# MegviiRobot/CamLaserCalibraTool

Hardware: NVIDIA H100
Metric: residual+Jacobian evals/sec (full LM solves) (higher is better)
Workload: dtype f64

## Files before the change

camlasercalibratool_b200/csrc/clc_api.cu:

```cuda
#include <cuda_runtime.h>
#include <dlfcn.h>
#include <nccl.h>

#include <algorithm>
#include <atomic>
#include <chrono>
#include <cmath>
#include <cstddef>
#include <cstdio>
#include <cstdlib>
#include <cstring>
#include <functional>
#include <mutex>
#include <string>
#include <vector>

#include "../../include/clc_b200.h"
#include "clc_kernels.cuh"
#include "clc_l2_plan.h"
#include "clc_linefit.cuh"
#include "clc_small.cuh"
#include "clc_subset.cuh"
#include "clc_subset_plan.h"
#include "clc_trim.cuh"
// ... 128 lines not shown
    if (piv != k) {
      for (int j = 0; j < n; ++j) std::swap(A[k * n + j], A[piv * n + j]);
      for (int j = 0; j < n; ++j) std::swap(A[j * n + k], A[j * n + piv]);
      std::swap(b[k], b[piv]);
      std::swap(perm[k], perm[piv]);
    }
    const double d = A[k * n + k];
    if (d == 0.0) continue;
    for (int i = k + 1; i < n; ++i) {
      const double l = A[i * n + k] / d;
      for (int j = k + 1; j < n; ++j) A[i * n + j] -= l * A[k * n + j];
      A[i * n + k] = l;
    }
  }
  double z[9], y[9];
  for (int i = 0; i < n; ++i) {
    double s = b[i];
    for (int k = 0; k < i; ++k) s -= A[i * n + k] * z[k];
    z[i] = s;
  }
  for (int i = 0; i < n; ++i) z[i] = (A[i * n + i] != 0.0) ? z[i] / A[i * n + i] : 0.0;
  for (int i = n - 1; i >= 0; --i) {
    double s = z[i];
    for (int k = i + 1; k < n; ++k) s -= A[k * n + i] * y[k];
    y[i] = s;
  }
  for (int i = 0; i < n; ++i) x[perm[i]] = y[i];
}

int64_t round_up(int64_t v, int64_t m) { return (v + m - 1) / m * m; }

}

struct PinnedBlock {
  clc::LmState lm;
  double sums[clc::kMaxOut];
  double pose[8];
  int done;
  int nonplanar;
};
namespace {
std::mutex g_pinned_mutex;
std::vector<PinnedBlock*> g_pinned_free;
PinnedBlock* pinned_acquire() {
  {
    std::lock_guard<std::mutex> lock(g_pinned_mutex);
    if (!g_pinned_free.empty()) {
      PinnedBlock* b = g_pinned_free.back();
      g_pinned_free.pop_back();
      return b;
    }
  }
  PinnedBlock* b = nullptr;
  if (cudaMallocHost(&b, sizeof(PinnedBlock)) != cudaSuccess) return nullptr;
  return b;
}
void pinned_release(PinnedBlock* b) {
  if (!b) return;
  std::lock_guard<std::mutex> lock(g_pinned_mutex);
  g_pinned_free.push_back(b);
}
}

struct clc_comm {
  ncclComm_t comm = nullptr;
  int nranks = 1, rank = 0, device = 0;
  void* p2p_block = nullptr;
  void* peer_block[clc::kMaxRanks] = {};
  bool p2p_ready = false;
  bool local = false;
  size_t mailbox_bytes() const { return sizeof(unsigned long long) * 2 * 2 * (size_t)nranks * clc::kMailboxSlot; }
  size_t block_bytes() const { return mailbox_bytes() + sizeof(unsigned long long); }
};

struct clc_problem {
  int device = 0;
  cudaStream_t stream = nullptr;
  int num_sms = 0;
  int64_t l2_bytes = 0;
  int grid = 0;
  int64_t n_frames = 0, n_points = 0, n_points_padded = 0, n_edges = 0;
  int use_loss = 1;
  double cauchy_a = 0.05;
  double *x = nullptr, *y = nullptr, *z = nullptr;
  void *xy_block = nullptr, *z_block = nullptr;
  double* frame_pose = nullptr;
  double* frame_pose_true = nullptr;
  double* plane = nullptr;
  int64_t* offsets = nullptr;
  int* warp_first_frame = nullptr;
  double* edge_plane = nullptr;
  double* edge_pt = nullptr;
  unsigned long long* partials_ll = nullptr;
  unsigned int* launch_seq = nullptr;
  unsigned long long* pose_ll = nullptr;
  double* sums = nullptr;
  double* pose = nullptr;
  clc::LmState* lm = nullptr;
  double* flush_buf = nullptr;
  int64_t flush_n = 0;
  unsigned long long* timing = nullptr;
  bool use_pdl = true;
  int64_t l2_persist_bytes = 0;
  bool l2_window_set = false;
  int64_t l2_resident_bytes = -1;
  int resident_chunks = 0;
  bool small_kernel = true;
  int loop_in_kernel = 1;
  PinnedBlock* pinned = nullptr;
  double* h_sums = nullptr;
  int* h_done = nullptr;
  clc::LmState* h_lm = nullptr;
  clc_comm* comm_obj = nullptr;
  ncclComm_t comm = nullptr;
  int nranks = 1, rank = 0;
  int* p2p_error = nullptr;
  int allreduce_mode = 0;
  int64_t per_warp = 0;
  int grid_full = 0;
  cudaEvent_t ev0 = nullptr, ev1 = nullptr;
  int* d_nonplanar = nullptr;
  bool z_all_zero = false;
  bool host_planarity_known = false;
  bool planar = false;
  int planar_mode = 1;
  int64_t planar_min_points = 0;
};

namespace {

clc::ProblemView make_view(const clc_problem* p) {
  clc::ProblemView v;
  v.x = p->x; v.y = p->y; v.z = p->z;
  v.plane = p->plane;
  v.offsets = p->offsets;
  v.warp_first_frame = p->warp_first_frame;
  v.edge_plane = p->edge_plane;
  v.edge_pt = p->edge_pt;
  v.n_frames = p->n_frames;
  v.n_points = p->n_points;
  v.n_edges = p->n_edges;
  v.per_warp = p->per_warp;
  v.resident_chunks = p->resident_chunks;
  v.a2 = p->cauchy_a * p->cauchy_a;
  v.inv_a2 = 1.0 / v.a2;
  return v;
}

int set_device(const clc_problem* p) {
  CLC_CUDA(cudaSetDevice(p->device));
  return CLC_OK;
}

int launch_sweep(clc_problem* p, int mode, bool loss, bool edges, const double* d_pose, const int* d_done,
                 clc::LmState* d_lm, bool collective = true, bool pdl = false, int loop_sweeps = 1, bool l2_hints = false,
                 double* frame_rows = nullptr, double* frame_slots = nullptr) {
  clc::SweepArgs a;
  a.pose7 = d_pose;
  a.done = d_done;
  a.partials_ll = p->partials_ll;
  a.sums = p->sums;
  a.launch_seq = p->launch_seq;
  a.pose_ll = p->pose_ll;
  a.lm = d_lm;
  a.use_loss = loss ? 1 : 0;
  a.use_edges = edges ? 1 : 0;
  a.l2_hints = l2_hints ? 1 : 0;
  a.loop_sweeps = loop_sweeps;
  a.timing = p->timing;
  a.nranks = 1;
  a.rank = 0;
  a.seq_counter = nullptr;
  a.error = p->p2p_error;
  a.frame_rows = frame_rows;
  a.frame_slots = frame_slots;
  if (p->nranks > 1 && p->allreduce_mode == 1 && collective) {
    clc_comm* c = p->comm_obj;
    a.nranks = c->nranks;
    a.rank = c->rank;
    a.seq_counter = reinterpret_cast<unsigned long long*>(static_cast<char*>(c->p2p_block) + c->mailbox_bytes());
    for (int r = 0; r < c->nranks; ++r) a.peer_mailbox[r] = static_cast<unsigned long long*>(c->peer_block[r]);
  }
  const clc::ProblemView v = make_view(p);
  cudaLaunchConfig_t cfg = {};
  cfg.gridDim = dim3((unsigned)p->grid);
  cfg.blockDim = dim3(clc::kThreads);
  cfg.dynamicSmemBytes = mode == clc::kModeFrames ? clc::frames_smem_bytes(p->planar) : clc::dyn_smem_bytes(p->planar);
  cfg.stream = p->stream;
  cudaLaunchAttribute attr[1];
  attr[0].id = cudaLaunchAttributeProgrammaticStreamSerialization;
  attr[0].val.programmaticStreamSerializationAllowed = pdl ? 1 : 0;
  cfg.attrs = attr;
  cfg.numAttrs = 1;
  cudaError_t le;
  if (!p->planar && p->z == nullptr) return fail(CLC_ERR_INVALID, "internal: general sweep without a z stream");
  if (mode == clc::kModeFrames) {
    if (frame_rows == nullptr || frame_slots == nullptr || d_lm != nullptr || loop_sweeps > 1 || a.nranks > 1)
      return fail(CLC_ERR_INVALID, "internal: bad per-frame sweep");
    void (*fn)(clc::ProblemView, clc::SweepArgs) =
        loss ? (p->planar ? clc::clc_sweep_kernel<true, clc::kModeFrames, true> : clc::clc_sweep_kernel<true, clc::kModeFrames, false>)
             : (p->planar ? clc::clc_sweep_kernel<false, clc::kModeFrames, true> : clc::clc_sweep_kernel<false, clc::kModeFrames, false>);
    CLC_CUDA(cudaFuncSetAttribute(fn, cudaFuncAttributeMaxDynamicSharedMemorySize, (int)cfg.dynamicSmemBytes));
    le = cudaLaunchKernelEx(&cfg, fn, v, a);
  } else if (mode == clc::kModeClosedForm) {
    le = p->planar ? cudaLaunchKernelEx(&cfg, clc::clc_sweep_kernel<false, clc::kModeClosedForm, true>, v, a)
                   : cudaLaunchKernelEx(&cfg, clc::clc_sweep_kernel<false, clc::kModeClosedForm, false>, v, a);
  } else if (loop_sweeps > 1) {
    if (d_lm == nullptr) return fail(CLC_ERR_INVALID, "internal: looping sweep without an LM state");
    if (loss)
      le = p->planar ? cudaLaunchKernelEx(&cfg, clc::clc_sweep_kernel<true, clc::kModeLM, true, true>, v, a)
                     : cudaLaunchKernelEx(&cfg, clc::clc_sweep_kernel<true, clc::kModeLM, false, true>, v, a);
    else
      le = p->planar ? cudaLaunchKernelEx(&cfg, clc::clc_sweep_kernel<false, clc::kModeLM, true, true>, v, a)
                     : cudaLaunchKernelEx(&cfg, clc::clc_sweep_kernel<false, clc::kModeLM, false, true>, v, a);
  } else if (loss) {
    le = p->planar ? cudaLaunchKernelEx(&cfg, clc::clc_sweep_kernel<true, clc::kModeLM, true>, v, a)
                   : cudaLaunchKernelEx(&cfg, clc::clc_sweep_kernel<true, clc::kModeLM, false>, v, a);
  } else {
    le = p->planar ? cudaLaunchKernelEx(&cfg, clc::clc_sweep_kernel<false, clc::kModeLM, true>, v, a)
                   : cudaLaunchKernelEx(&cfg, clc::clc_sweep_kernel<false, clc::kModeLM, false>, v, a);
  }
  if (le != cudaSuccess) return fail(CLC_ERR_CUDA, std::string("sweep launch: ") + cudaGetErrorString(le));
  CLC_LAUNCH_CHECK();
  return CLC_OK;
}

int allreduce_sums(clc_problem* p, int count) {
  if (p->nranks <= 1 || p->allreduce_mode == 1) return CLC_OK;
  CLC_NCCL(nccl_api()->AllReduce(p->sums, p->sums, (size_t)count, ncclDouble, ncclSum, p->comm, p->stream));
  return CLC_OK;
}

cudaError_t sync_stream_low_latency(cudaStream_t st) {
  const auto t0 = std::chrono::steady_clock::now();
  for (;;) {
    const cudaError_t e = cudaStreamQuery(st);
    if (e != cudaErrorNotReady) return e;
    if (std::chrono::steady_clock::now() - t0 > std::chrono::microseconds(400)) return cudaStreamSynchronize(st);
#if defined(__x86_64__) || defined(__i386__)
    __builtin_ia32_pause();
#endif
  }
}

int check_p2p_error(clc_problem* p) {
  if (p->grid <= 1 && p->nranks <= 1) return CLC_OK;
  int err = 0;
  CLC_CUDA(cudaMemcpyAsync(&err, p->p2p_error, sizeof(int), cudaMemcpyDeviceToHost, p->stream));
  CLC_CUDA(sync_stream_low_latency(p->stream));
  if (err == 2) return fail(CLC_ERR_CUDA, "sweep kernel: the persistent grid was not co-resident (ticket wait timed out)");
  if (err) return fail(CLC_ERR_NCCL, "peer exchange timed out: a rank did not reach the collective");
  return CLC_OK;
}

int materialise_z(clc_problem* p);

int partition(clc_problem* p) {
  const int chunk = p->planar ? clc::kPlanarChunk : clc::kChunk;
  p->grid = p->grid_full;
  {
    const int64_t stages = (p->n_points + chunk - 1) / chunk;
    const int64_t blocks_needed = std::max<int64_t>(1, (stages + clc::kWarps - 1) / clc::kWarps);
    if (blocks_needed < p->grid) p->grid = (int)blocks_needed;
    int64_t single_block_max = (int64_t)clc::kWarps * 8 * clc::kChunk;
    if (const char* env = std::getenv("CLC_SINGLE_BLOCK_MAX_POINTS")) single_block_max = std::atoll(env);
    if (p->n_points <= single_block_max) p->grid = 1;
  }
  const int64_t n_warps = (int64_t)p->grid * clc::kWarps;
  p->per_warp = std::max<int64_t>(chunk, round_up((p->n_points + n_warps - 1) / n_warps, chunk));
  if (p->warp_first_frame) CLC_CUDA(cudaFreeAsync(p->warp_first_frame, p->stream));
  if (p->partials_ll) CLC_CUDA(cudaFreeAsync(p->partials_ll, p->stream));
  p->warp_first_frame = nullptr;
  p->partials_ll = nullptr;
  CLC_CUDA(cudaMallocAsync(&p->warp_first_frame, sizeof(int) * n_warps, p->stream));
  const size_t ll_bytes = sizeof(unsigned long long) * 2 * (size_t)p->grid * clc::kMaxOut;
  CLC_CUDA(cudaMallocAsync(&p->partials_ll, ll_bytes, p->stream));
  {
    const int64_t stage_bytes = (int64_t)(p->planar ? 2 : 3) * chunk * 8;
    const bool latency_bound = p->n_points <= clc::kSmallMaxResiduals;
    const int64_t budget = p->l2_persist_bytes > 0 ? 0 : clc::l2_resident_budget(p->l2_bytes, p->l2_resident_bytes);
    p->resident_chunks = clc::l2_resident_chunks(budget, p->grid, clc::kWarps, p->per_warp / chunk, stage_bytes, latency_bound);
  }
  CLC_CUDA(cudaMemsetAsync(p->partials_ll, 0, ll_bytes, p->stream));
  const int threads = 256;
  const int blocks = (int)((n_warps + threads - 1) / threads);
  clc::clc_warp_table_kernel<<<blocks, threads, 0, p->stream>>>(p->offsets, p->n_frames, p->n_points, p->per_warp, n_warps,
                                                                p->warp_first_frame);
  CLC_LAUNCH_CHECK();
  return CLC_OK;
}

int finish_create(clc_problem* p) {
  const int threads = 256;
  if (p->n_frames > 0) {
    const int blocks = (int)((p->n_frames + threads - 1) / threads);
    clc::clc_planes_kernel<<<blocks, threads, 0, p->stream>>>(p->frame_pose, p->n_frames, p->plane, p->edge_plane);
    CLC_LAUNCH_CHECK();
  }
  static std::mutex cfg_mutex;
  static int cached_blocks_per_sm[64] = {};
  int blocks_per_sm = 0;
  {
    std::lock_guard<std::mutex> lock(cfg_mutex);
    if (p->device < 64) blocks_per_sm = cached_blocks_per_sm[p->device];
  }
  if (blocks_per_sm == 0) {
    int occ = 0, occ_min = 1 << 30;
    const void* variants[] = {
        (const void*)clc::clc_sweep_kernel<true, clc::kModeLM, false>,         (const void*)clc::clc_sweep_kernel<true, clc::kModeLM, true>,
        (const void*)clc::clc_sweep_kernel<false, clc::kModeLM, false>,        (const void*)clc::clc_sweep_kernel<false, clc::kModeLM, true>,
        (const void*)clc::clc_sweep_kernel<false, clc::kModeClosedForm, false>, (const void*)clc::clc_sweep_kernel<false, clc::kModeClosedForm, true>,
        (const void*)clc::clc_sweep_kernel<true, clc::kModeLM, false, true>,   (const void*)clc::clc_sweep_kernel<true, clc::kModeLM, true, true>,
        (const void*)clc::clc_sweep_kernel<false, clc::kModeLM, false, true>,  (const void*)clc::clc_sweep_kernel<false, clc::kModeLM, true, true>};
    for (int v = 0; v < 10; ++v) {
      const void* fn = variants[v];
      const int smem = clc::dyn_smem_bytes((v & 1) != 0);
      CLC_CUDA(cudaFuncSetAttribute(fn, cudaFuncAttributeMaxDynamicSharedMemorySize, smem));
      CLC_CUDA(cudaOccupancyMaxActiveBlocksPerMultiprocessor(&occ, fn, clc::kThreads, smem));
      occ_min = std::min(occ_min, occ);
    }
    if (occ_min < 1) return fail(CLC_ERR_CUDA, "the sweep kernel does not fit on this device");
// ... 2345 lines not shown
```

camlasercalibratool_b200/csrc/clc_kernels.cuh:

```cuda
#pragma once

#include <cuda_runtime.h>

#include "clc_camera.cuh"
#include "clc_expand.cuh"
#include "clc_frames.cuh"
#include "clc_lm.cuh"

namespace clc {

#ifndef CLC_THREADS
#define CLC_THREADS 384
#endif
#ifndef CLC_BLOCKS_PER_SM
#define CLC_BLOCKS_PER_SM 1
#endif
#ifndef CLC_STAGES
#define CLC_STAGES 2
#endif
constexpr int kThreads = CLC_THREADS;
constexpr int kBlocksPerSM = CLC_BLOCKS_PER_SM;
constexpr int kWarps = kThreads / 32;
constexpr int kTileStride = 13;
#ifndef CLC_CHUNK
#define CLC_CHUNK 128
#endif
constexpr int kChunk = CLC_CHUNK;
constexpr int kGroups = kChunk / 64;
constexpr int kStages = CLC_STAGES;
constexpr int kMaxOut = 54;
constexpr int kMaxRanks = 16;
constexpr int kMailboxSlot = 64;
#ifndef CLC_PLANAR_STAGES
#define CLC_PLANAR_STAGES CLC_STAGES
#endif
#ifndef CLC_PLANAR_CHUNK
#define CLC_PLANAR_CHUNK (CLC_CHUNK * 2)
#endif
constexpr int kPlanarStages = CLC_PLANAR_STAGES;
constexpr int kPlanarChunk = CLC_PLANAR_CHUNK;
static_assert(kChunk % 64 == 0 && kPlanarChunk % 64 == 0, "stages are made of 64-point groups");
constexpr int kMaxChunk = kChunk > kPlanarChunk ? kChunk : kPlanarChunk;
#ifndef CLC_LOCKSTEP_SLACK
#define CLC_LOCKSTEP_SLACK 0
#endif
constexpr int kLockstepSlack = CLC_LOCKSTEP_SLACK;
constexpr int kBarsPerWarp = kStages > kPlanarStages ? kStages : kPlanarStages;
constexpr int kTileDoublesPerWarp = 32 * kTileStride;
__host__ __device__ constexpr int ring_doubles_per_warp(bool planar) { return planar ? kPlanarStages * 2 * kPlanarChunk : kStages * 3 * kChunk; }
__host__ __device__ constexpr int dyn_smem_bytes(bool planar) {
  return kWarps * ring_doubles_per_warp(planar) * 8 + kWarps * kTileDoublesPerWarp * 8 + kWarps * kBarsPerWarp * 8;
}

constexpr int kFrameTileDoublesPerWarp = 32 * 3;
__host__ __device__ constexpr int frames_smem_bytes(bool planar) {
  return dyn_smem_bytes(planar) + kWarps * kFrameTileDoublesPerWarp * 8;
}

enum SweepMode { kModeLM = 0, kModeClosedForm = 1, kModeFrames = 2 };

struct ProblemView {
  const double* x;
  const double* y;
  const double* z;
  const double* plane;
  const int64_t* offsets;
  const int* warp_first_frame;
  const double* edge_plane;
  const double* edge_pt;
  int64_t n_frames;
  int64_t n_points;
  int64_t n_edges;
  int64_t per_warp;
  int resident_chunks;
  double inv_a2;
  double a2;
};

struct SweepArgs {
  const double* pose7;
  const int* done;
  unsigned long long* partials_ll;
  double* sums;
  unsigned int* launch_seq;
  LmState* lm;
  int use_loss;
  int use_edges;
  int l2_hints;
  int loop_sweeps;
  unsigned long long* pose_ll;
  unsigned long long* timing;
  int nranks;
  int rank;
  unsigned long long* seq_counter;
  unsigned long long* peer_mailbox[kMaxRanks];
  int* error;
  double* frame_rows;
  double* frame_slots;
};


__device__ __forceinline__ unsigned long long globaltimer_ns() {
  unsigned long long t;
  asm volatile("mov.u64 %0, %globaltimer;" : "=l"(t));
  return t;
}
#define CLC_STAMP(slot)                                                                       \
  do {                                                                                        \
    if (args.timing != nullptr && threadIdx.x == 0) args.timing[(int64_t)blockIdx.x * 8 + (slot)] = globaltimer_ns(); \
  } while (0)

__device__ __forceinline__ uint32_t smem_u32(const void* p) { return (uint32_t)__cvta_generic_to_shared(p); }

__device__ __forceinline__ void mbar_init(uint64_t* bar, uint32_t count) {
  asm volatile("mbarrier.init.shared::cta.b64 [%0], %1;" ::"r"(smem_u32(bar)), "r"(count) : "memory");
}
__device__ __forceinline__ void mbar_expect_tx(uint64_t* bar, uint32_t bytes) {
  asm volatile("mbarrier.arrive.expect_tx.shared::cta.b64 _, [%0], %1;" ::"r"(smem_u32(bar)), "r"(bytes) : "memory");
}
__device__ __forceinline__ void mbar_wait(uint64_t* bar, uint32_t parity) {
  uint32_t done;
  do {
    asm volatile(
        "{\n\t.reg .pred p;\n\t"
        "mbarrier.try_wait.parity.shared::cta.b64 p, [%1], %2;\n\t"
        "selp.u32 %0, 1, 0, p;\n\t}"
        : "=r"(done)
        : "r"(smem_u32(bar)), "r"(parity)
        : "memory");
  } while (!done);
}
__device__ __forceinline__ void bulk_g2s(void* dst, const void* src, uint32_t bytes, uint64_t* bar) {
  asm volatile("cp.async.bulk.shared::cluster.global.mbarrier::complete_tx::bytes [%0], [%1], %2, [%3];" ::"r"(
                   smem_u32(dst)),
               "l"(src), "r"(bytes), "r"(smem_u32(bar))
               : "memory");
}
__device__ __forceinline__ void bulk_g2s_hint(void* dst, const void* src, uint32_t bytes, uint64_t* bar, uint64_t policy) {
  asm volatile("cp.async.bulk.shared::cluster.global.mbarrier::complete_tx::bytes.L2::cache_hint [%0], [%1], %2, [%3], %4;" ::"r"(
                   smem_u32(dst)),
               "l"(src), "r"(bytes), "r"(smem_u32(bar)), "l"(policy)
               : "memory");
}
__device__ __forceinline__ uint64_t policy_evict_last() {
  uint64_t pol;
  asm("createpolicy.fractional.L2::evict_last.b64 %0, 1.0;" : "=l"(pol));
  return pol;
}
__device__ __forceinline__ uint64_t policy_evict_first() {
  uint64_t pol;
  asm("createpolicy.fractional.L2::evict_first.b64 %0, 1.0;" : "=l"(pol));
  return pol;
}

__device__ __forceinline__ void st_relaxed_sys(unsigned long long* p, unsigned long long v) {
  asm volatile("st.relaxed.sys.global.u64 [%0], %1;" ::"l"(p), "l"(v) : "memory");
}
__device__ __forceinline__ unsigned long long ld_relaxed_sys(const unsigned long long* p) {
  unsigned long long v;
  asm volatile("ld.relaxed.sys.global.u64 %0, [%1];" : "=l"(v) : "l"(p) : "memory");
  return v;
}

__device__ __forceinline__ void st_volatile_v2(unsigned long long* p, unsigned long long a, unsigned long long b) {
  asm volatile("st.volatile.global.v2.u64 [%0], {%1, %2};" ::"l"(p), "l"(a), "l"(b) : "memory");
}
__device__ __forceinline__ void ld_volatile_v2(const unsigned long long* p, unsigned long long& a, unsigned long long& b) {
  asm volatile("ld.volatile.global.v2.u64 {%0, %1}, [%2];" : "=l"(a), "=l"(b) : "l"(p) : "memory");
}

__device__ __forceinline__ unsigned int ld_acquire_gpu(const unsigned int* p) {
  unsigned int v;
  asm volatile("ld.acquire.gpu.global.u32 %0, [%1];" : "=r"(v) : "l"(p) : "memory");
  return v;
}
__device__ __forceinline__ unsigned int atom_add_acq_rel_gpu(unsigned int* p, unsigned int v) {
  unsigned int old;
  asm volatile("atom.acq_rel.gpu.global.add.u32 %0, [%1], %2;" : "=r"(old) : "l"(p), "r"(v) : "memory");
  return old;
}

__device__ __forceinline__ double rcp_pos(double a) {
  double r;
  asm("rcp.approx.ftz.f64 %0, %1;" : "=d"(r) : "d"(a));
  double e = fma(-a, r, 1.0);
  r = fma(r, e, r);
  e = fma(-a, r, 1.0);
  r = fma(r, e, r);
  return r;
}

__device__ __forceinline__ double warp_sum(double v) {
#pragma unroll
  for (int o = 16; o > 0; o >>= 1) v += __shfl_xor_sync(0xffffffffu, v, o);
  return v;
}

template <int N>
__device__ __forceinline__ void warp_transpose_sum(double* v, int lane) {
#pragma unroll
  for (int half = N / 2; half >= 1; half >>= 1) {
    const bool upper = (lane & half) != 0;
#pragma unroll
    for (int i = 0; i < half; ++i) {
      const double keep = upper ? v[i + half] : v[i];
      const double send = upper ? v[i] : v[i + half];
      v[i] = keep + __shfl_xor_sync(0xffffffffu, send, half);
    }
  }
#pragma unroll
  for (int o = N; o < 32; o <<= 1) v[0] += __shfl_xor_sync(0xffffffffu, v[0], o);
}

struct Moments {
  double S0, Sx, Sy, Sz, Sxx, Sxy, Sxz, Syy, Syz, Szz;
  double prod;
  int esum;
};

template <bool LOSS>
__device__ __forceinline__ void moments_clear(Moments& a) {
  a.S0 = a.Sx = a.Sy = a.Sz = a.Sxx = a.Sxy = a.Sxz = a.Syy = a.Syz = a.Szz = 0.0;
  a.prod = LOSS ? 1.0 : 0.0;
  a.esum = 0;
}

template <bool PLANAR>
__device__ __forceinline__ void accumulate(Moments& a, double w, double x, double y, double z) {
  const double wx = w * x, wy = w * y;
  a.S0 += w;
  a.Sx += wx; a.Sy += wy;
  a.Sxx = fma(wx, x, a.Sxx); a.Sxy = fma(wx, y, a.Sxy);
  a.Syy = fma(wy, y, a.Syy);
  if (!PLANAR) {
    const double wz = w * z;
    a.Sz += wz;
    a.Sxz = fma(wx, z, a.Sxz); a.Syz = fma(wy, z, a.Syz); a.Szz = fma(wz, z, a.Szz);
  }
}

template <bool LOSS, bool COST, bool PLANAR>
__device__ __forceinline__ void process2(Moments& a, const double2 X, const double2 Y, const double2 Z, bool v0,
                                         bool v1, double m0, double m1, double m2, double c, double inv_a2) {
  const double e0 = fma(m0, X.x, fma(m1, Y.x, PLANAR ? c : fma(m2, Z.x, c)));
  const double e1 = fma(m0, X.y, fma(m1, Y.y, PLANAR ? c : fma(m2, Z.y, c)));
  if (LOSS) {
    double u0 = fma(e0 * inv_a2, e0, 1.0);
    double u1 = fma(e1 * inv_a2, e1, 1.0);
    u0 = v0 ? u0 : 1.0;
    u1 = v1 ? u1 : 1.0;
    const double p = u0 * u1;
    const double r = rcp_pos(p);
    double w0 = r * u1, w1 = r * u0;
    w0 = v0 ? w0 : 0.0;
    w1 = v1 ? w1 : 0.0;
    a.prod *= p;
    accumulate<PLANAR>(a, w0, X.x, Y.x, Z.x);
    accumulate<PLANAR>(a, w1, X.y, Y.y, Z.y);
  } else {
    if (COST) {
      a.prod = fma(v0 ? e0 : 0.0, e0, a.prod);
      a.prod = fma(v1 ? e1 : 0.0, e1, a.prod);
    }
    accumulate<PLANAR>(a, v0 ? 1.0 : 0.0, X.x, Y.x, Z.x);
    accumulate<PLANAR>(a, v1 ? 1.0 : 0.0, X.y, Y.y, Z.y);
  }
}

__device__ __forceinline__ void renormalise(Moments& a) {
  const int hi = __double2hiint(a.prod);
  const int ex = (hi >> 20) - 1023;
  a.esum += ex;
  a.prod = __hiloint2double(hi - (ex << 20), __double2loint(a.prod));
}

struct FrameSums {
  double se, se2, emax;
};

__device__ __forceinline__ void frame_sums_clear(FrameSums& s) { s.se = s.se2 = s.emax = 0.0; }

template <bool PLANAR>
__device__ __forceinline__ void frame_sums2(FrameSums& s, const double2 X, const double2 Y, const double2 Z, bool v0, bool v1,
                                            double m0, double m1, double m2, double c) {
  const double e0 = fma(m0, X.x, fma(m1, Y.x, PLANAR ? c : fma(m2, Z.x, c)));
  const double e1 = fma(m0, X.y, fma(m1, Y.y, PLANAR ? c : fma(m2, Z.y, c)));
  const double d0 = v0 ? e0 : 0.0, d1 = v1 ? e1 : 0.0;
  s.se += d0;
  s.se += d1;
  s.se2 = fma(d0, d0, s.se2);
  s.se2 = fma(d1, d1, s.se2);
  s.emax = nan_max(s.emax, fabs(d0));
  s.emax = nan_max(s.emax, fabs(d1));
}

__device__ __forceinline__ void frame_row_write(const ProblemView& pv, const PoseConsts& pc, int64_t f, int64_t n, const double* S,
                                                double cost_term, double se, double se2, double emax, bool loss, bool edges,
                                                double* row) {
  double plane[4], m[3], c;
#pragma unroll
  for (int k = 0; k < 4; ++k) plane[k] = pv.plane[f * 4 + k];
  frame_consts(pc, plane, m, &c);
  const double s2 = 1.0 / (double)(pv.offsets[f + 1] - pv.offsets[f]);
  double out[kNumSums];
#pragma unroll
  for (int k = 0; k < kNumSums; ++k) out[k] = 0.0;
  expand_lm(plane, m, c, s2, S, loss, cost_term, pv.a2, out);
  double ee[2] = {0.0, 0.0};
  if (edges) {
#pragma unroll
    for (int k = 0; k < 2; ++k)
      ee[k] = edge_residual(pc, pv.edge_plane + (2 * f + k) * 4, pv.edge_pt + (2 * f + k) * 3, s2, loss, pv.a2, pv.inv_a2, out);
  }
  const double dn = (double)n;
  row[kRowN] = __longlong_as_double(n);
  row[kRowCost] = out[27];
  row[kRowChi] = s2 * se2;
  row[kRowMeanE] = se / dn;
  row[kRowRmsE] = sqrt(se2 / dn);
  row[kRowMaxE] = emax;
  row[kRowMeanW] = S[0] / dn;
  row[kRowEdgeE] = ee[0];
  row[kRowEdgeE + 1] = ee[1];
#pragma unroll
  for (int k = 0; k < 21; ++k) row[kRowH + k] = out[k];
#pragma unroll
  for (int k = 0; k < 6; ++k) row[kRowG + k] = out[21 + k];
}

template <bool LOSS, int MODE, bool PLANAR, bool LOOP = false>
__global__ void __launch_bounds__(kThreads, kBlocksPerSM)
clc_sweep_kernel(ProblemView pv, SweepArgs args) {
  constexpr int NOUT = (MODE == kModeClosedForm) ? kMaxOut : kNumSums;
  constexpr int NST = PLANAR ? kPlanarStages : kStages;
  constexpr int CH = PLANAR ? kPlanarChunk : kChunk;
  constexpr int G = CH / 64;
  constexpr int SST = (PLANAR ? 2 : 3) * CH;
  constexpr int RING = NST * SST;
  static_assert(RING == ring_doubles_per_warp(PLANAR), "ring size");
  extern __shared__ __align__(128) unsigned char s_dyn[];
  __shared__ double s_acc[kWarps][NOUT];
  __shared__ double s_red[kWarps][32];
  __shared__ unsigned long long s_core[kLmCoreWords];
  __shared__ double s_next[8];
  __shared__ int s_prog[32];

  CLC_STAMP(0);
  if (args.timing != nullptr && threadIdx.x == 0) {
    unsigned int smid;
    asm volatile("mov.u32 %0, %smid;" : "=r"(smid));
    args.timing[(int64_t)blockIdx.x * 8 + 7] = smid;
  }

  const int lane = threadIdx.x & 31;
  const int warp = threadIdx.x >> 5;
  const int64_t gwarp = (int64_t)blockIdx.x * kWarps + warp;

  const int64_t P = pv.n_points;
  int64_t p0 = gwarp * pv.per_warp;
  if (p0 > P) p0 = P;
  int64_t p1 = p0 + pv.per_warp;
  if (p1 > P) p1 = P;
  const int n_chunks = (int)((p1 - p0 + CH - 1) / CH);
  double* ring = reinterpret_cast<double*>(s_dyn) + warp * RING;
  double* tile = reinterpret_cast<double*>(s_dyn) + kWarps * RING + warp * kTileDoublesPerWarp;
  uint64_t* bars = reinterpret_cast<uint64_t*>(s_dyn + (size_t)kWarps * (RING + kTileDoublesPerWarp) * 8) + warp * kBarsPerWarp;
  double* ftile = reinterpret_cast<double*>(s_dyn + dyn_smem_bytes(PLANAR)) + warp * kFrameTileDoublesPerWarp;

  const int sweeps_max = (LOOP && args.loop_sweeps > 1 && MODE == kModeLM && args.lm != nullptr) ? args.loop_sweeps : 1;
  const int total_chunks = LOOP ? sweeps_max * n_chunks : n_chunks;
  int issued = 0, next_c = 0;
  const bool l2_hints = args.l2_hints != 0 && pv.resident_chunks > 0;
  auto issue_one = [&](bool slot_was_read) {
    if (lane == 0) {
      const int c = LOOP ? next_c : issued, st = issued % NST;
      double* dst = ring + st * SST;
      const int64_t src = p0 + (int64_t)c * CH;
      if (slot_was_read) asm volatile("fence.proxy.async.shared::cta;" ::: "memory");
      mbar_expect_tx(bars + st, (PLANAR ? 2 : 3) * CH * 8);
      if (l2_hints) {
        const uint64_t pol = c >= n_chunks - pv.resident_chunks ? policy_evict_last() : policy_evict_first();
        bulk_g2s_hint(dst, pv.x + src, CH * 8, bars + st, pol);
        bulk_g2s_hint(dst + CH, pv.y + src, CH * 8, bars + st, pol);
        if (!PLANAR) bulk_g2s_hint(dst + 2 * CH, pv.z + src, CH * 8, bars + st, pol);
      } else {
        bulk_g2s(dst, pv.x + src, CH * 8, bars + st);
        bulk_g2s(dst + CH, pv.y + src, CH * 8, bars + st);
        if (!PLANAR) bulk_g2s(dst + 2 * CH, pv.z + src, CH * 8, bars + st);
      }
    }
    ++issued;
    if (LOOP && ++next_c == n_chunks) next_c = 0;
  };
  auto drain = [&](int g) {
    for (; g < issued; ++g) mbar_wait(bars + g % NST, (uint32_t)(g / NST) & 1u);
  };
  if (lane == 0) {
#pragma unroll
    for (int st = 0; st < NST; ++st) mbar_init(bars + st, 1);
    asm volatile("fence.mbarrier_init.release.cluster;" ::: "memory");
    asm volatile("fence.proxy.async.shared::cta;" ::: "memory");
  }
  __syncwarp();
  for (int g = 0; g < NST && g < total_chunks; ++g) issue_one(false);
  __syncwarp();

  asm volatile("griddepcontrol.wait;" ::: "memory");
  if (args.done != nullptr && (*args.done != 0 || (args.error != nullptr && *args.error != 0))) {
    drain(0);
    return;
  }

  const unsigned int launch_tag0 = *args.launch_seq + 1u;
  if (MODE == kModeLM && args.lm != nullptr && blockIdx.x == 0) {
    const unsigned long long* g_core = reinterpret_cast<const unsigned long long*>(&args.lm->core);
    for (int k = threadIdx.x; k < kLmCoreWords; k += kThreads) s_core[k] = __ldcg(g_core + k);
  }

  PoseConsts pc;
  int n_tile = 0;

  auto flush_tile = [&]() {
    double out[NOUT];
#pragma unroll
    for (int k = 0; k < NOUT; ++k) out[k] = 0.0;
    __syncwarp();
    if (lane < n_tile) {
      const double* row = tile + lane * kTileStride;
      const int64_t f = __double_as_longlong(row[12]);
      double plane[4];
#pragma unroll
      for (int k = 0; k < 4; ++k) plane[k] = pv.plane[f * 4 + k];
      if (MODE == kModeLM) {
        double m[3], c;
        frame_consts(pc, plane, m, &c);
        const double cnt = (double)(pv.offsets[f + 1] - pv.offsets[f]);
        double cost_term = row[10];
        if (LOSS) cost_term = log(row[10]) + row[11] * 0.693147180559945309417232121458;
        expand_lm(plane, m, c, 1.0 / cnt, row, LOSS, cost_term, pv.a2, out);
      } else {
        expand_closed_form(plane, row, out);
      }
    }
    {
      double v[32];
#pragma unroll
      for (int k = 0; k < 32; ++k) v[k] = (k < NOUT) ? out[k] : 0.0;
      warp_transpose_sum<32>(v, lane);
      if (lane < NOUT) s_acc[warp][lane] += v[0];
      if (NOUT > 32) {
#pragma unroll
        for (int k = 0; k < 32; ++k) v[k] = (32 + k < NOUT) ? out[(32 + k < NOUT) ? 32 + k : 0] : 0.0;
        warp_transpose_sum<32>(v, lane);
        if (32 + lane < NOUT) s_acc[warp][32 + lane] += v[0];
      }
    }
    __syncwarp();
    n_tile = 0;
  };

  auto flush_frames = [&]() {
    __syncwarp();
    if (lane < n_tile) {
      const double* row = tile + lane * kTileStride;
      const double* rx = ftile + lane * 3;
      const int64_t f = __double_as_longlong(row[12]);
      const double cost_term = LOSS ? log(row[10]) + row[11] * 0.693147180559945309417232121458 : rx[1];
      frame_row_write(pv, pc, f, pv.offsets[f + 1] - pv.offsets[f], row, cost_term, rx[0], rx[1], rx[2], LOSS,
                      args.use_edges && pv.n_edges > 0, args.frame_rows + f * kRowDoubles);
    }
    __syncwarp();
    n_tile = 0;
  };

  int gc_base = 0;
  for (int sw = 0;; ++sw) {
  const unsigned int launch_tag = LOOP ? launch_tag0 + (unsigned int)sw : launch_tag0;
  for (int k = lane; k < NOUT; k += 32) s_acc[warp][k] = 0.0;
  {
    double pose[7];
#pragma unroll
    for (int i = 0; i < 7; ++i) pose[i] = (LOOP && sw > 0) ? s_next[i] : args.pose7[i];
    make_pose_consts(pose, &pc);
  }

  if (kLockstepSlack > 0) {
    if (lane == 0) s_prog[warp] = n_chunks > 0 ? 0 : 0x7fffffff;
    if (warp == 0 && lane >= kWarps) s_prog[lane] = 0x7fffffff;
    __syncthreads();
  }
  if (n_chunks > 0) {
    int64_t f = pv.warp_first_frame[gwarp];
    int64_t f_end = pv.offsets[f + 1];
    double m0 = 0.0, m1 = 0.0, m2 = 0.0, c = 0.0;
    double nx_plane[4] = {0.0, 0.0, 0.0, 0.0};
    int64_t nx_end = 0;
    auto prefetch_next = [&]() {
      if (f + 1 < pv.n_frames) {
#pragma unroll
        for (int k = 0; k < 4; ++k) nx_plane[k] = pv.plane[(f + 1) * 4 + k];
        nx_end = pv.offsets[f + 2];
      }
    };
    auto set_frame_consts = [&](const double* plane) {
      double m[3];
      frame_consts(pc, plane, m, &c);
      m0 = m[0]; m1 = m[1]; m2 = m[2];
    };
    {
      double plane[4];
#pragma unroll
      for (int k = 0; k < 4; ++k) plane[k] = pv.plane[f * 4 + k];
      set_frame_consts(plane);
      prefetch_next();
    }
    Moments a;
    moments_clear<LOSS>(a);
    bool open = false;
    FrameSums fx;
    frame_sums_clear(fx);
    int64_t piece_n = 0;

    auto park_piece = [&]() {
      double v[16] = {a.S0, a.Sx, a.Sy, a.Sz, a.Sxx, a.Sxy, a.Sxz, a.Syy, a.Syz, a.Szz, 0.0, 0.0, 0.0, 0.0, 0.0, 0.0};
      double pr = a.prod;
      int es = a.esum;
      double em = 0.0;
      if (MODE == kModeFrames) {
        v[12] = fx.se;
        v[13] = fx.se2;
        em = fx.emax;
#pragma unroll
        for (int o = 16; o > 0; o >>= 1) em = nan_max(em, __shfl_xor_sync(0xffffffffu, em, o));
      }
      if (LOSS) {
#pragma unroll
        for (int o = 16; o > 0; o >>= 1) {
          pr *= __shfl_xor_sync(0xffffffffu, pr, o);
          es += __shfl_xor_sync(0xffffffffu, es, o);
        }
      } else {
        v[10] = pr;
      }
      warp_transpose_sum<16>(v, lane);
      const int kind = MODE == kModeFrames ? frame_piece_kind(pv.offsets[f], f_end, p0, p1) : (int)kPieceWhole;
      if (kind != kPieceWhole) {
        double* slot = args.frame_slots + (gwarp * 2 + (kind == kPieceHead ? kSlotHead : kSlotTail)) * kSlotDoubles;
        if (lane < 10 || lane == 12 || lane == 13) slot[lane] = v[0];
        if (lane == 10) slot[10] = LOSS ? pr : 0.0;
        if (lane == 11) slot[11] = (double)es;
        if (lane == 14) slot[14] = em;
        if (lane == 15) slot[15] = (double)piece_n;
      } else {
        {
          double* row = tile + n_tile * kTileStride;
          if (lane < 10 || (!LOSS && lane == 10)) row[lane] = v[0];
          if (LOSS && lane == 10) row[10] = pr;
          if (lane == 11) row[11] = (double)es;
          if (lane == 12) row[12] = __longlong_as_double(f);
        }
        if (MODE == kModeFrames) {
          double* rx = ftile + n_tile * 3;
          if (lane == 12) rx[0] = v[0];
          if (lane == 13) rx[1] = v[0];
          if (lane == 14) rx[2] = em;
        }
        ++n_tile;
        if (n_tile == 32) {
          if (MODE == kModeFrames) flush_frames();
          else flush_tile();
        }
      }
      moments_clear<LOSS>(a);
      open = false;
      if (MODE == kModeFrames) {
        frame_sums_clear(fx);
        piece_n = 0;
      }
    };

    for (int ch = 0; ch < n_chunks; ++ch) {
      const int gc = LOOP ? gc_base + ch : ch;
      const int st = gc % NST;
      const int64_t cb = p0 + (int64_t)ch * CH;
      const int64_t ce = (cb + CH < p1) ? cb + CH : p1;
      if (kLockstepSlack > 0) {
        while (__reduce_min_sync(0xffffffffu, *(volatile int*)&s_prog[lane]) < ch - kLockstepSlack) __nanosleep(40);
      }
      mbar_wait(bars + st, (uint32_t)(gc / NST) & 1u);
      const double* sx = ring + st * SST;
      double2 X[G], Y[G], Z[G];
#pragma unroll
      for (int g = 0; g < G; ++g) {
        X[g] = *reinterpret_cast<const double2*>(sx + 64 * g + 2 * lane);
        Y[g] = *reinterpret_cast<const double2*>(sx + CH + 64 * g + 2 * lane);
        Z[g] = PLANAR ? make_double2(0.0, 0.0) : *reinterpret_cast<const double2*>(sx + 2 * CH + 64 * g + 2 * lane);
      }
      int64_t q = cb;
      while (q < ce) {
        while (f_end <= q) {
          ++f;
          if (nx_end > q) {
            f_end = nx_end;
            set_frame_consts(nx_plane);
          } else {
            f_end = pv.offsets[f + 1];
            if (f_end > q) {
              double plane[4];
#pragma unroll
              for (int k = 0; k < 4; ++k) plane[k] = pv.plane[f * 4 + k];
              set_frame_consts(plane);
            }
          }
          if (f_end > q) prefetch_next();
          else nx_end = 0;
        }
        const int64_t hi = f_end < ce ? f_end : ce;
        if (q == cb && hi == cb + CH) {
#pragma unroll
          for (int g = 0; g < G; ++g) {
            process2<LOSS, MODE == kModeLM, PLANAR>(a, X[g], Y[g], Z[g], true, true, m0, m1, m2, c, pv.inv_a2);
            if (MODE == kModeFrames) frame_sums2<PLANAR>(fx, X[g], Y[g], Z[g], true, true, m0, m1, m2, c);
          }
        } else {
#pragma unroll
          for (int g = 0; g < G; ++g) {
            const int64_t i0 = cb + 64 * g + 2 * lane;
            process2<LOSS, MODE == kModeLM, PLANAR>(a, X[g], Y[g], Z[g], i0 >= q && i0 < hi, i0 + 1 >= q && i0 + 1 < hi, m0, m1, m2,
                                            c, pv.inv_a2);
            if (MODE == kModeFrames)
              frame_sums2<PLANAR>(fx, X[g], Y[g], Z[g], i0 >= q && i0 < hi, i0 + 1 >= q && i0 + 1 < hi, m0, m1, m2, c);
          }
        }
        if (LOSS) renormalise(a);
        open = true;
        if (MODE == kModeFrames) piece_n += hi - q;
        q = hi;
        if (hi == f_end) park_piece();
      }
      __syncwarp();
      if (issued < total_chunks) issue_one(true);
      if (kLockstepSlack > 0 && lane == 0) *(volatile int*)&s_prog[warp] = (ch + 1 == n_chunks) ? 0x7fffffff : ch + 1;
    }
    if (open) park_piece();
  }
  if (MODE == kModeFrames) {
    flush_frames();
    return;
  }
  CLC_STAMP(1);
  if (args.timing != nullptr && lane == 0) args.timing[(int64_t)gridDim.x * 8 + gwarp] = globaltimer_ns();
  flush_tile();
  CLC_STAMP(2);

  if (MODE == kModeLM && args.use_edges && pv.n_edges > 0) {
    const int64_t total_lanes = (int64_t)gridDim.x * kThreads;
    double out[NOUT];
#pragma unroll
    for (int k = 0; k < NOUT; ++k) out[k] = 0.0;
    bool any = false;
    for (int64_t i = gwarp * 32 + lane; i < pv.n_edges; i += total_lanes) {
      const int64_t f = i >> 1;
      const int64_t cnt = pv.offsets[f + 1] - pv.offsets[f];
      if (cnt <= 0) continue;
      any = true;
      double plane[4], m[3], c;
#pragma unroll
      for (int k = 0; k < 4; ++k) plane[k] = pv.edge_plane[i * 4 + k];
      frame_consts(pc, plane, m, &c);
      const double x = pv.edge_pt[i * 3], y = pv.edge_pt[i * 3 + 1], z = pv.edge_pt[i * 3 + 2];
      const double e = fma(m[0], x, fma(m[1], y, fma(m[2], z, c)));
      double w = 1.0, cost_term = e * e;
      if (LOSS) {
        const double u = fma(e * pv.inv_a2, e, 1.0);
        w = 1.0 / u;
        cost_term = log(u);
      }
      const double S[10] = {w, w * x, w * y, w * z, w * x * x, w * x * y, w * x * z, w * y * y, w * y * z, w * z * z};
      expand_lm(plane, m, c, 1.0 / (double)cnt, S, LOSS, cost_term, pv.a2, out);
    }
    if (__any_sync(0xffffffffu, any)) {
      double v[32];
#pragma unroll
      for (int k = 0; k < 32; ++k) v[k] = (k < NOUT) ? out[k] : 0.0;
      warp_transpose_sum<32>(v, lane);
      if (lane < NOUT) s_acc[warp][lane] += v[0];
      __syncwarp();
    }
  }

  const unsigned long long ll_tag = (unsigned long long)launch_tag << 32;
  __syncthreads();
  double block_sum = 0.0;
  if (threadIdx.x < NOUT) {
#pragma unroll
    for (int wv = 0; wv < kWarps; ++wv) block_sum += s_acc[wv][threadIdx.x];
    if (gridDim.x > 1) {
      const unsigned long long bits = (unsigned long long)__double_as_longlong(block_sum);
      st_volatile_v2(args.partials_ll + ((int64_t)blockIdx.x * kMaxOut + threadIdx.x) * 2, ll_tag | (bits & 0xffffffffull),
                     ll_tag | (bits >> 32));
    }
  }
  CLC_STAMP(3);
  asm volatile("griddepcontrol.launch_dependents;" ::: "memory");
  if (blockIdx.x != 0 && (!LOOP || sweeps_max == 1)) return;

  if (blockIdx.x == 0) {
    constexpr int PARTS = kThreads / NOUT;
    constexpr int NB = 10;
    double* s_gather = &s_red[0][0];
    static_assert(kWarps * 32 >= PARTS * NOUT, "s_red holds one value per gathering thread");
    if (gridDim.x > 1 && threadIdx.x < PARTS * NOUT) {
      const int k = threadIdx.x % NOUT, part = threadIdx.x / NOUT;
      double acc = 0.0;
      for (int base = part; base < (int)gridDim.x; base += PARTS * NB) {
        unsigned long long w0[NB], w1[NB];
        unsigned int pending = 0u;
#pragma unroll
        for (int u = 0; u < NB; ++u)
          if (base + u * PARTS < (int)gridDim.x) pending |= 1u << u;
        unsigned int polls = 0;
        unsigned long long t0 = 0;
        while (pending != 0u) {
#pragma unroll
          for (int u = 0; u < NB; ++u)
            if ((pending >> u) & 1u)
              ld_volatile_v2(args.partials_ll + ((int64_t)(base + u * PARTS) * kMaxOut + k) * 2, w0[u], w1[u]);
#pragma unroll
          for (int u = 0; u < NB; ++u)
            if (((pending >> u) & 1u) && (w0[u] & 0xffffffff00000000ull) == ll_tag && (w1[u] & 0xffffffff00000000ull) == ll_tag)
              pending &= ~(1u << u);
          if (pending != 0u && (++polls & 0xffu) == 0u) {
            const unsigned long long now = globaltimer_ns();
            if (t0 == 0) t0 = now;
            else if (now - t0 > 2000000000ull) {
              if (args.error != nullptr) *args.error = 2;
              break;
            }
          }
        }
#pragma unroll
        for (int u = 0; u < NB; ++u)
          if (base + u * PARTS < (int)gridDim.x) acc += __longlong_as_double((long long)((w1[u] << 32) | (w0[u] & 0xffffffffull)));
      }
      s_gather[threadIdx.x] = acc;
    }
    double total = block_sum;
    if (gridDim.x > 1) {
      __syncthreads();
      total = 0.0;
      if (threadIdx.x < NOUT) {
#pragma unroll
        for (int part = 0; part < PARTS; ++part) total += s_gather[part * NOUT + threadIdx.x];
      }
    }
    if (args.nranks > 1) {
      double* s_tot = s_acc[0];
      double* s_x = reinterpret_cast<double*>(s_dyn) + kWarps * RING;
      static_assert(kWarps * kTileDoublesPerWarp >= kMaxRanks * kMaxOut, "the tiles hold one value per rank and output");
      __syncthreads();
      if (threadIdx.x < NOUT) s_tot[threadIdx.x] = total;
      __syncthreads();
      const unsigned long long seq = *args.seq_counter + 1ull;
      const unsigned long long tag = (seq & 0xffffffffull) << 32;
      const int par = (int)(seq & 1ull);
      const int n_words = args.nranks * NOUT;
      for (int idx = threadIdx.x; idx < n_words; idx += kThreads) {
        const int r = idx / NOUT, k = idx % NOUT;
        const unsigned long long bits = (unsigned long long)__double_as_longlong(s_tot[k]);
        const int64_t slot = (((int64_t)par * args.nranks + args.rank) * kMailboxSlot + k) * 2;
        st_relaxed_sys(args.peer_mailbox[r] + slot, tag | (bits & 0xffffffffull));
        st_relaxed_sys(args.peer_mailbox[r] + slot + 1, tag | (bits >> 32));
      }
      const unsigned long long t0 = globaltimer_ns();
      for (int idx = threadIdx.x; idx < n_words; idx += kThreads) {
        const int r = idx / NOUT, k = idx % NOUT;
        const unsigned long long* src = args.peer_mailbox[args.rank] + (((int64_t)par * args.nranks + r) * kMailboxSlot + k) * 2;
        unsigned long long a0, a1;
        unsigned int polls = 0;
        for (;;) {
          a0 = ld_relaxed_sys(src);
          a1 = ld_relaxed_sys(src + 1);
          if ((a0 & 0xffffffff00000000ull) == tag && (a1 & 0xffffffff00000000ull) == tag) break;
          if ((++polls & 0x3fu) == 0u && globaltimer_ns() - t0 > 5000000000ull) {
            if (args.error != nullptr) *args.error = 1;
            break;
          }
        }
        s_x[idx] = __longlong_as_double((long long)((a1 << 32) | (a0 & 0xffffffffull)));
      }
      __syncthreads();
      if (threadIdx.x < NOUT) {
        total = 0.0;
        for (int r = 0; r < args.nranks; ++r) total += s_x[r * NOUT + threadIdx.x];
      }
      if (threadIdx.x == 0) *args.seq_counter = seq;
    }
    __syncthreads();
    if (threadIdx.x < NOUT) {
      args.sums[threadIdx.x] = total;
      if (threadIdx.x < 32) s_red[0][threadIdx.x] = total;
    }
    __syncthreads();
    CLC_STAMP(4);
    if (threadIdx.x == 0) *args.launch_seq = launch_tag;
    if (MODE == kModeLM && args.lm != nullptr) {
      if (threadIdx.x == 0) {
        double sums[kNumSums];
        for (int k = 0; k < kNumSums; ++k) sums[k] = s_red[0][k];
        if (args.error != nullptr && *args.error != 0) {
          reinterpret_cast<LmCore*>(s_core)->done = CLC_TERM_FAILURE;
        } else {
          lm_update(reinterpret_cast<LmCore*>(s_core), args.lm->trace, sums);
        }
      }
      __syncthreads();
      if (LOOP && sweeps_max > 1 && threadIdx.x < 8) {
        const LmCore* core = reinterpret_cast<const LmCore*>(s_core);
        const double v = threadIdx.x < 7 ? core->cand[threadIdx.x] : (double)core->done;
        s_next[threadIdx.x] = v;
        if (gridDim.x > 1) {
          const unsigned long long bits = (unsigned long long)__double_as_longlong(v);
          st_volatile_v2(args.pose_ll + 2 * threadIdx.x, ll_tag | (bits & 0xffffffffull), ll_tag | (bits >> 32));
        }
      }
      unsigned long long* o_core = reinterpret_cast<unsigned long long*>(&args.lm->core);
      for (int k = threadIdx.x; k < kLmCoreWords; k += kThreads) o_core[k] = s_core[k];
    }
    CLC_STAMP(5);
  } else {
    if (threadIdx.x < 8 && sw + 1 < sweeps_max) {
      unsigned long long a0, a1, t0 = 0;
      unsigned int polls = 0;
      for (;;) {
        ld_volatile_v2(args.pose_ll + 2 * threadIdx.x, a0, a1);
        if ((a0 & 0xffffffff00000000ull) == ll_tag && (a1 & 0xffffffff00000000ull) == ll_tag) break;
        if ((++polls & 0xffu) == 0u) {
          const unsigned long long now = globaltimer_ns();
          if (t0 == 0) t0 = now;
          else if (now - t0 > 10000000000ull) {
            if (args.error != nullptr) *args.error = 2;
            a0 = a1 = 0;
            break;
          }
        }
      }
      const bool lost = (a0 | a1) == 0ull;
      s_next[threadIdx.x] = lost ? (double)CLC_TERM_FAILURE : __longlong_as_double((long long)((a1 << 32) | (a0 & 0xffffffffull)));
    }
  }
  if (!LOOP || sw + 1 >= sweeps_max) break;
  gc_base += n_chunks;
  __syncthreads();
  if (s_next[7] != 0.0) {
    drain(gc_base);
    break;
  }
  }
}

__global__ void clc_lm_kernel(LmState* lm, const double* sums) {
  if (threadIdx.x == 0 && blockIdx.x == 0) {
    double s[kNumSums];
    for (int k = 0; k < kNumSums; ++k) s[k] = sums[k];
    lm_update(&lm->core, lm->trace, s);
  }
}

template <bool LOSS>
__global__ void clc_frame_fixup_kernel(ProblemView pv, const double* pose7, int edges, const double* __restrict__ slots,
                                       double* __restrict__ rows) {
  const int64_t f = (int64_t)blockIdx.x * blockDim.x + threadIdx.x;
  if (f >= pv.n_frames) return;
  const int64_t fs = pv.offsets[f], fe = pv.offsets[f + 1];
  double* row = rows + f * kRowDoubles;
  if (fe <= fs) {
    for (int k = 0; k < kRowDoubles; ++k) row[k] = 0.0;
    return;
  }
  int64_t w0, w1;
  frame_warps(fs, fe, pv.per_warp, &w0, &w1);
  if (w0 == w1) return;
  double S[10] = {0.0, 0.0, 0.0, 0.0, 0.0, 0.0, 0.0, 0.0, 0.0, 0.0};
  double cost_term = 0.0, se = 0.0, se2 = 0.0, emax = 0.0;
  int64_t n = 0;
  for (int64_t w = w0; w <= w1; ++w) {
    const double* s = slots + frame_slot(w, w0);
#pragma unroll
    for (int k = 0; k < 10; ++k) S[k] += s[k];
    cost_term += LOSS ? log(s[10]) + s[11] * 0.693147180559945309417232121458 : s[13];
    se += s[12];
    se2 += s[13];
    emax = nan_max(emax, s[14]);
    n += (int64_t)s[15];
  }
  PoseConsts pc;
  make_pose_consts(pose7, &pc);
  frame_row_write(pv, pc, f, n, S, cost_term, se, se2, emax, LOSS, edges != 0, row);
}


__global__ void clc_aos_to_soa_kernel(const double* __restrict__ aos, int64_t n, double* __restrict__ x,
                                      double* __restrict__ y, double* __restrict__ z, int64_t dst_off,
                                      int* __restrict__ nonplanar) {
  const int64_t i = (int64_t)blockIdx.x * blockDim.x + threadIdx.x;
  bool off_plane = false;
  if (i < n) {
    x[dst_off + i] = aos[3 * i];
    y[dst_off + i] = aos[3 * i + 1];
    const double zi = aos[3 * i + 2];
    z[dst_off + i] = zi;
    off_plane = !(zi == 0.0);
  }
  if (__any_sync(0xffffffffu, off_plane) && (threadIdx.x & 31) == 0) atomicOr(nonplanar, 1);
}

__global__ void clc_aos2_to_soa_kernel(const double2* __restrict__ xy, int64_t n, double* __restrict__ x,
                                       double* __restrict__ y, double* __restrict__ z, int64_t dst_off) {
  const int64_t i = (int64_t)blockIdx.x * blockDim.x + threadIdx.x;
  if (i < n) {
    const double2 v = xy[i];
    x[dst_off + i] = v.x;
    y[dst_off + i] = v.y;
    if (z != nullptr) z[dst_off + i] = 0.0;
  }
}

__global__ void clc_soa_to_aos_kernel(const double* __restrict__ x, const double* __restrict__ y,
                                      const double* __restrict__ z, int64_t src_off, int64_t n,
                                      double* __restrict__ aos) {
  const int64_t i = (int64_t)blockIdx.x * blockDim.x + threadIdx.x;
  if (i < n) {
    aos[3 * i] = x[src_off + i];
    aos[3 * i + 1] = y[src_off + i];
    aos[3 * i + 2] = (z != nullptr) ? z[src_off + i] : 0.0;
  }
}

__global__ void clc_planes_kernel(const double* __restrict__ frame_pose, int64_t n_frames, double* __restrict__ plane,
                                  double* __restrict__ edge_plane) {
  const int64_t f = (int64_t)blockIdx.x * blockDim.x + threadIdx.x;
  if (f >= n_frames) return;
  double fp[7], pl[4];
  for (int k = 0; k < 7; ++k) fp[k] = frame_pose[f * 7 + k];
  frame_plane(fp, pl);
  for (int k = 0; k < 4; ++k) plane[f * 4 + k] = pl[k];
  if (edge_plane != nullptr) {
    double p1[4], p2[4];
    edge_planes(fp, p1, p2);
    for (int k = 0; k < 4; ++k) {
      edge_plane[(2 * f) * 4 + k] = p1[k];
      edge_plane[(2 * f + 1) * 4 + k] = p2[k];
    }
  }
}

__global__ void clc_warp_table_kernel(const int64_t* __restrict__ offsets, int64_t n_frames, int64_t n_points,
                                      int64_t per_warp, int64_t n_warps, int* __restrict__ first_frame) {
  const int64_t w = (int64_t)blockIdx.x * blockDim.x + threadIdx.x;
  if (w >= n_warps) return;
  const int64_t p0 = w * per_warp;
  if (p0 >= n_points) { first_frame[w] = 0; return; }
  int64_t lo = 0, hi = n_frames;
  while (hi - lo > 1) {
// ... 97 lines not shown
```

Measured before the change: 91.90 billion.

## Release PDL dependents early and hoist frame-head loads before grid dependency wait

When PDL is on and the sweep is single-shot, single-rank and the point data fits under a size cap, the kernel issues griddepcontrol.launch_dependents before griddepcontrol.wait so the next launch can start its prologue sooner. For non-loop LM mode, the warp's first-frame metadata and plane loads are moved ahead of the dependency wait to hide their latency. In loop mode the LM update is called through a noinline wrapper, likely to reduce register pressure or code size. The early-release path depends on dependents not reading data before their own wait, so correctness rests on the PDL ordering.

```diff
diff --git a/camlasercalibratool_b200/csrc/clc_api.cu b/camlasercalibratool_b200/csrc/clc_api.cu
--- a/camlasercalibratool_b200/csrc/clc_api.cu
+++ b/camlasercalibratool_b200/csrc/clc_api.cu
@@ -304,6 +304,8 @@
   return CLC_OK;
 }
 
+constexpr int64_t kEarlyReleaseMaxBytes = (int64_t)1 << 30;
+
 int launch_sweep(clc_problem* p, int mode, bool loss, bool edges, const double* d_pose, const int* d_done,
                  clc::LmState* d_lm, bool collective = true, bool pdl = false, int loop_sweeps = 1, bool l2_hints = false,
                  double* frame_rows = nullptr, double* frame_slots = nullptr) {
@@ -319,6 +321,7 @@
   a.use_edges = edges ? 1 : 0;
   a.l2_hints = l2_hints ? 1 : 0;
   a.loop_sweeps = loop_sweeps;
+  a.early_release = pdl && loop_sweeps <= 1 && p->nranks <= 1 && p->n_points * (p->planar ? 16 : 24) <= kEarlyReleaseMaxBytes ? 1 : 0;
   a.timing = p->timing;
   a.nranks = 1;
   a.rank = 0;
diff --git a/camlasercalibratool_b200/csrc/clc_kernels.cuh b/camlasercalibratool_b200/csrc/clc_kernels.cuh
--- a/camlasercalibratool_b200/csrc/clc_kernels.cuh
+++ b/camlasercalibratool_b200/csrc/clc_kernels.cuh
@@ -87,6 +87,7 @@
   int use_loss;
   int use_edges;
   int l2_hints;
+  int early_release;
   int loop_sweeps;
   unsigned long long* pose_ll;
   unsigned long long* timing;
@@ -328,6 +329,8 @@
   for (int k = 0; k < 6; ++k) row[kRowG + k] = out[21 + k];
 }
 
+__device__ __noinline__ void lm_update_out_of_line(LmCore* s, clc_lm_iteration* trace, const double* sums) { lm_update(s, trace, sums); }
+
 template <bool LOSS, int MODE, bool PLANAR, bool LOOP = false>
 __global__ void __launch_bounds__(kThreads, kBlocksPerSM)
 clc_sweep_kernel(ProblemView pv, SweepArgs args) {
@@ -405,6 +408,27 @@
   for (int g = 0; g < NST && g < total_chunks; ++g) issue_one(false);
   __syncwarp();
 
+  constexpr bool HEAD_EARLY = !LOOP && MODE == kModeLM;
+  int64_t head_f = 0, head_end = 0, head_nx_end = 0;
+  double head_plane[4], head_nx_plane[4];
+  auto load_head = [&]() {
+    head_f = pv.warp_first_frame[gwarp];
+    head_end = pv.offsets[head_f + 1];
+    head_nx_end = 0;
+#pragma unroll
+    for (int k = 0; k < 4; ++k) {
+      head_plane[k] = pv.plane[head_f * 4 + k];
+      head_nx_plane[k] = 0.0;
+    }
+    if (head_f + 1 < pv.n_frames) {
+#pragma unroll
+      for (int k = 0; k < 4; ++k) head_nx_plane[k] = pv.plane[(head_f + 1) * 4 + k];
+      head_nx_end = pv.offsets[head_f + 2];
+    }
+  };
+  if (HEAD_EARLY && n_chunks > 0) load_head();
+
+  if (args.early_release) asm volatile("griddepcontrol.launch_dependents;" ::: "memory");
   asm volatile("griddepcontrol.wait;" ::: "memory");
   if (args.done != nullptr && (*args.done != 0 || (args.error != nullptr && *args.error != 0))) {
     drain(0);
@@ -490,11 +514,12 @@
     __syncthreads();
   }
   if (n_chunks > 0) {
-    int64_t f = pv.warp_first_frame[gwarp];
-    int64_t f_end = pv.offsets[f + 1];
+    if (!HEAD_EARLY) load_head();
+    int64_t f = head_f;
+    int64_t f_end = head_end;
     double m0 = 0.0, m1 = 0.0, m2 = 0.0, c = 0.0;
-    double nx_plane[4] = {0.0, 0.0, 0.0, 0.0};
-    int64_t nx_end = 0;
+    double nx_plane[4] = {head_nx_plane[0], head_nx_plane[1], head_nx_plane[2], head_nx_plane[3]};
+    int64_t nx_end = head_nx_end;
     auto prefetch_next = [&]() {
       if (f + 1 < pv.n_frames) {
 #pragma unroll
@@ -507,13 +532,7 @@
       frame_consts(pc, plane, m, &c);
       m0 = m[0]; m1 = m[1]; m2 = m[2];
     };
-    {
-      double plane[4];
-#pragma unroll
-      for (int k = 0; k < 4; ++k) plane[k] = pv.plane[f * 4 + k];
-      set_frame_consts(plane);
-      prefetch_next();
-    }
+    set_frame_consts(head_plane);
     Moments a;
     moments_clear<LOSS>(a);
     bool open = false;
@@ -810,6 +829,8 @@
         for (int k = 0; k < kNumSums; ++k) sums[k] = s_red[0][k];
         if (args.error != nullptr && *args.error != 0) {
           reinterpret_cast<LmCore*>(s_core)->done = CLC_TERM_FAILURE;
+        } else if (LOOP) {
+          lm_update_out_of_line(reinterpret_cast<LmCore*>(s_core), args.lm->trace, sums);
         } else {
           lm_update(reinterpret_cast<LmCore*>(s_core), args.lm->trace, sums);
         }
```

After: 94.00 billion, median of 6. +2.3%, better.
